# Neos-codes/microbeast

Measured on AMD Instinct MI355X. Metric: env frames/sec (whole node) on 16x16 microRTS, higher is better.
Workload: dtype bf16

## Files before the change

### microbeast_amd/_native.py

```python
from __future__ import annotations

import ctypes
import importlib.util
import os
import sys
import threading
from pathlib import Path

import torch

_LIB = Path(__file__).resolve().parent / "_lib"
_lock = threading.Lock()
_kern = None
_rt = None

c_void_p, c_int, c_int64, c_float = ctypes.c_void_p, ctypes.c_int, ctypes.c_int64, ctypes.c_float

_SIGS = {
    "mbk_multi_copy": [c_void_p, c_int, c_void_p],
    "mbk_comm_standin": [c_void_p, c_void_p, c_int64, c_int, c_int, c_void_p],
    "mbk_row_gather": [c_void_p, c_void_p, c_void_p, c_int, c_int64, c_void_p],
    "mbk_memset": [c_void_p, c_int, c_int64, c_void_p],
    "mbk_masked_cell_fwd": [c_void_p, c_int, c_void_p, c_void_p, c_void_p, c_int, c_int64,
                            c_void_p, c_void_p, c_void_p],
# ... 53 lines not shown
    "mbk_set_learner_occupancy": [c_int, c_int],
    "mbk_set_work_queues": [c_int],
    "mbk_set_work_queue_site": [c_int, c_int],
    "mbk_conv0_row_set": [c_int],
    "mbk_fc_wgrad_parts": [c_int, c_int, c_int],
    "mbk_fc_wgrad": [c_void_p, c_void_p, c_int, c_int, c_int, c_void_p, c_int, c_void_p, c_int,
                     c_void_p],
    "mbk_fc_fwd": [c_void_p, c_int, c_void_p, c_void_p, c_void_p, c_void_p, c_int, c_int, c_int,
                   c_void_p, c_void_p, c_void_p],
    "mbk_gemm_nt": [c_void_p, c_void_p, c_void_p, c_void_p, c_int, c_int, c_int, c_int, c_int,
                    c_int, c_int, c_int, c_int, c_void_p],
    "mbk_wgrad_reduce": [c_void_p, c_int, c_int, c_int, c_int, c_void_p, c_void_p, c_int,
                         c_void_p],
    "mbk_wgrad_reduce_batch": [c_void_p, c_int, c_void_p],
    "mbk_pool_bwd": [c_void_p, c_void_p, c_int, c_int, c_int, c_int, c_void_p, c_void_p],
    "mbk_conv_pack": [c_void_p, c_int, c_void_p],
    "mbk_head_compact": [c_void_p, c_int, c_int, c_void_p, c_void_p, c_void_p, c_void_p,
                         c_void_p, c_void_p, c_void_p, c_void_p, c_void_p, c_void_p, c_void_p,
                         c_void_p, c_void_p, c_int, c_void_p, c_void_p, c_void_p, c_void_p],
    "mbk_head_fwd": [c_void_p, c_void_p, c_void_p, c_void_p, c_void_p, c_void_p, c_int,
                     c_void_p, c_void_p, c_void_p, c_void_p, c_void_p, c_void_p, c_int, c_int,
                     c_void_p, c_void_p, c_int, c_void_p],
    "mbk_fc_wgrad_wide_parts": [c_int, c_int, c_int],
    "mbk_fc_wgrad_wide": [c_void_p, c_void_p, c_int, c_int, c_int, c_int, c_void_p, c_int,
                          c_void_p, c_void_p, c_void_p],
    "mbk_head_score": [c_void_p, c_void_p, c_void_p, c_void_p, c_void_p, c_void_p, c_void_p,
                       c_void_p, c_void_p, c_void_p, c_void_p, c_int, c_void_p, c_void_p,
                       c_void_p, c_void_p],
    "mbk_head_pair_rowsum": [c_void_p, c_void_p, c_int, c_int, c_void_p, c_void_p, c_void_p,
                             c_void_p, c_void_p],
    "mbk_head_bwd": [c_void_p, c_void_p, c_void_p, c_void_p, c_void_p, c_void_p, c_void_p,
                     c_void_p, c_void_p, c_void_p, c_void_p, c_void_p, c_void_p, c_void_p,
                     c_void_p, c_int, c_int, c_void_p, c_void_p, c_void_p, c_void_p,
                     c_void_p, c_void_p, c_void_p],
    "mbk_head_dx_gather": [c_void_p, c_void_p, c_void_p, c_int, c_int, c_void_p, c_void_p],
    "mbk_head_dx_value_parts": [c_int],
    "mbk_head_dx_value": [c_void_p, c_void_p, c_void_p, c_int, c_int, c_void_p, c_void_p,
                          c_void_p, c_int, c_void_p, c_void_p, c_int, c_void_p],
    "mbk_head_pack": [c_void_p, c_void_p, c_int, c_void_p, c_void_p, c_void_p, c_void_p],
    "mbk_decode_obs_mask": [c_void_p, c_void_p, c_int, c_int, c_int, c_void_p, c_void_p, c_void_p],
    "mbk_decode_obs_mask_bucket": [c_void_p, c_void_p, c_int, c_int, c_int, c_void_p, c_void_p,
                                   c_void_p, c_void_p, c_void_p, c_void_p, c_void_p],
    "mbk_head_units": [c_void_p, c_int, c_int, c_void_p, c_void_p, c_void_p, c_void_p, c_void_p,
                       c_void_p],
    "mbk_row_sum_rng": [c_void_p, c_int64, c_int, c_void_p, c_void_p, c_void_p],
    "mbk_row_sum_pack": [c_void_p, c_int64, c_int, c_void_p, c_void_p, c_void_p, c_void_p,
                         c_void_p, c_int, c_void_p],
    "mbk_head_fwd_counts": [c_void_p, c_void_p, c_void_p, c_void_p, c_void_p, c_void_p,
                            c_void_p, c_void_p, c_int, c_int, c_int, c_void_p, c_void_p],
    "mbk_trunk_tail": [c_void_p, c_void_p, c_void_p, c_int, c_int, c_int, c_void_p, c_void_p],
    "mbk_trunk_tail_fp8": [c_void_p, c_void_p, c_void_p, c_void_p, c_int, c_int, c_int, c_void_p,
                           c_void_p],
    "mbk_trunk_tail_fc": [c_void_p, c_void_p, c_void_p, c_int, c_int, c_int, c_void_p, c_void_p,
                          c_void_p, c_void_p, c_void_p, c_int, c_void_p, c_void_p, c_void_p],
    "mbk_pack_env_actions": [c_void_p, c_int64, c_void_p, c_void_p],
    "mbk_res_bwd16_parts": [c_int, c_int, c_int, c_int],
    "mbk_res_bwd32_parts": [c_int, c_int, c_int, c_int],
    "mbk_res_bwd32_partial_floats": [c_int],
    "mbk_res_bwd32": [c_void_p, c_void_p, c_void_p, c_void_p, c_void_p, c_void_p, c_void_p, c_int,
                      c_void_p, c_void_p, c_void_p, c_void_p, c_int, c_int, c_int, c_int,
                      c_int, c_void_p],
    "mbk_res_fwd16": [c_void_p, c_void_p, c_void_p, c_void_p, c_void_p, c_void_p, c_void_p, c_int,
                      c_int, c_int, c_int, c_void_p],
    "mbk_res_fwd16_stage": [c_void_p, c_void_p, c_void_p, c_void_p, c_void_p, c_void_p, c_void_p,
                            c_void_p, c_void_p, c_void_p, c_void_p, c_int, c_int, c_int, c_int,
                            c_void_p],
    "mbk_res_blk32_fwd": [c_void_p, c_void_p, c_void_p, c_void_p, c_void_p, c_int, c_int, c_int, c_int,
# ... 118 lines not shown
```

### microbeast_amd/csrc/kernels/head.hip

```cpp
#include <cstdio>
#include <vector>

#include "../include/mbk_api.h"
#include "../include/microrts_rules.h"
#include "common.h"

#ifndef MBK_HA_MB
#define MBK_HA_MB 4
#endif

using namespace mbk;

typedef __bf16 bf16x8 __attribute__((ext_vector_type(8)));
typedef short s16x4 __attribute__((ext_vector_type(4)));
typedef float f32x4 __attribute__((ext_vector_type(4)));
typedef __hip_bfloat16 bf16;

namespace {

constexpr int KD = 256;
constexpr int NP = 80;
constexpr int NPT = 96;

union Frag8 {
// ... 510 lines not shown
  }
}
__global__ __launch_bounds__(64 * HA_NW, 2) void head_act_kernel(HeadActArgs a) {
  head_act_kernel_body(a);
}

__global__ __launch_bounds__(256) void head_pair_rowsum_kernel(const int* __restrict__ pidx,
                                                               const uint32_t* __restrict__ abits,
                                                               int F,
                                                               int S, const float* __restrict__ plp,
                                                               const float* __restrict__ pent,
                                                               float* __restrict__ logp,
                                                               float* __restrict__ ent) {
  const int f = blockIdx.x * 256 + threadIdx.x;
  if (f >= F) return;
  const int SW = abits_words(S);
  const uint32_t* ab = abits + (size_t)f * SW;
  const int* pr = pidx + (size_t)f * S;
  float a = 0.f, b = 0.f;
  for (int w = 0; w < SW; ++w) {
    uint32_t bits = ab[w];
    if (32 * w + 32 > S) bits &= (1u << (S - 32 * w)) - 1u;
    while (bits) {
      const int p = pr[32 * w + __builtin_ctz(bits)];
      bits &= bits - 1u;
      a += plp[p];
      if (pent) b += pent[p];
    }
  }
  logp[f] = a;
  if (ent) ent[f] = b;
}

constexpr int HB_NW = 8;
constexpr int HB_TM = 16 * HB_NW;
constexpr int HB_RX = 544, HB_RW = 544, HB_RZ = 288;
constexpr int HB_LW = 0, HB_LX = 96 * HB_RW, HB_LZ = HB_LX + HB_TM * HB_RX;
constexpr int HB_LB = HB_LZ + HB_TM * HB_RZ;
constexpr int HB_LDS = HB_LB + HB_NW * NP * 4;

__device__ __forceinline__ int hb_phi(int r) {
  const int b = (r >> 2) & 3;
  return (b == 1 || b == 2) ? r ^ 12 : r;
}
template <int CTRL>
__device__ __forceinline__ float hb_dpp(float v) {
  return __int_as_float(__builtin_amdgcn_mov_dpp(__float_as_int(v), CTRL, 0xF, 0xF, true));
}
constexpr int kHbDpp[4] = {0xB1, 0x4E, 0x141, 0x140};
template <int N>
__device__ __forceinline__ void hb_max16(float (&v)[N]) {
#pragma unroll
  for (int st = 0; st < 4; ++st)
#pragma unroll
    for (int j = 0; j < N; ++j) {
      const float o = st == 0 ? hb_dpp<0xB1>(v[j]) : st == 1 ? hb_dpp<0x4E>(v[j])
                    : st == 2 ? hb_dpp<0x141>(v[j]) : hb_dpp<0x140>(v[j]);
      v[j] = fmaxf(v[j], o);
    }
}
template <int N>
__device__ __forceinline__ void hb_sum16(float (&v)[N]) {
#pragma unroll
  for (int st = 0; st < 4; ++st)
#pragma unroll
    for (int j = 0; j < N; ++j) {
      const float o = st == 0 ? hb_dpp<0xB1>(v[j]) : st == 1 ? hb_dpp<0x4E>(v[j])
                    : st == 2 ? hb_dpp<0x141>(v[j]) : hb_dpp<0x140>(v[j]);
      v[j] += o;
    }
}

template <bool ST>
__global__ __launch_bounds__(64 * HB_NW, 1) void head_bwd2_kernel(
    const bf16* __restrict__ X, const bf16* __restrict__ Wp, const float* __restrict__ bp,
    const uint32_t* __restrict__ mask, const uint8_t* __restrict__ action,
    const int* __restrict__ pairs, const int* __restrict__ grp_start,
    const int* __restrict__ grp_count, const int* __restrict__ chunk_cell,
    const int* __restrict__ chunk_row, const int* __restrict__ totals,
    const float* __restrict__ g_logp, const float* __restrict__ g_ent, int S,
    bf16* __restrict__ dXp, float* __restrict__ dWp, float* __restrict__ dbp,
    uint64_t* __restrict__ stamps, const float* __restrict__ stats) {
  extern __shared__ __attribute__((aligned(16))) char smem[];
  char* wl = smem + HB_LW;
  int nst = 0;
#define HB_STAMP(k)                                                                        \
  do {                                                                                     \
    if (stamps && threadIdx.x == 0 && nst < 8)                                             \
      stamps[((size_t)blockIdx.x * 8 + nst) * 8 + (k)] = __builtin_amdgcn_s_memrealtime(); \
  } while (0)
  char* xl = smem + HB_LX;
  char* zl = smem + HB_LZ;
  float* bl = (float*)(smem + HB_LB);
  const int tid = threadIdx.x, lane = tid & 63, wave = tid >> 6;
  const int G = lane >> 4, li = lane & 15;
  const int nchunks = totals[2];
  const int qn = (nchunks + (int)gridDim.x - 1) / (int)gridDim.x;
  const int ch_begin = (int)blockIdx.x * qn, ch_end = min(nchunks, ch_begin + qn);
  if (ch_begin >= nchunks) return;
  for (int e = tid; e < 16 * HB_RW / 16; e += 64 * HB_NW)
    ((uint4*)(wl + 80 * HB_RW))[e] = make_uint4(0, 0, 0, 0);

  int sk[5], so[5];
#pragma unroll
  for (int nb = 0; nb < 5; ++nb) {
    const int col = nb * 16 + li;
    int k = 0;
#pragma unroll
    for (int q = 1; q < kComps; ++q) k += col >= seg_off(q) ? 1 : 0;
    sk[nb] = col < kCell ? k : kComps;
    so[nb] = col - seg_off(k);
  }

  const int sq = tid & 31, sr0 = tid >> 5;
  uint4 xr[8];
  struct Cur {
    int ch, t0, c, g0, n;
  };
  auto chunk_cur = [&](int ch) {
    if (ch >= ch_end) ch = nchunks;
    Cur u{ch, 0, 0, 0, 0};
    if (ch < nchunks) {
      u.c = chunk_cell[ch];
      u.g0 = chunk_row[ch];
      u.n = min(CHUNK, grp_start[u.c] + grp_count[u.c] - u.g0);
    }
    return u;
  };
  auto advance = [&](const Cur& u) {
    if (u.ch >= nchunks) return u;
    if (u.t0 + HB_TM < u.n) return Cur{u.ch, u.t0 + HB_TM, u.c, u.g0, u.n};
    return chunk_cur(u.ch + 1);
  };
  const int mrow = tid / 3, mpart = tid - 3 * (tid / 3);
  int fx[8], fr = -1;
  uint32_t mt[3] = {0u, 0u, 0u};
  auto load_fx = [&](const Cur& u) {
    const int nr = u.ch < nchunks ? min(HB_TM, u.n - u.t0) : 0;
#pragma unroll
    for (int k = 0; k < 8; ++k) fx[k] = sr0 + 16 * k < nr ? pairs[u.g0 + u.t0 + sr0 + 16 * k] : -1;
    fr = tid < 3 * HB_TM && mrow < nr ? pairs[u.g0 + u.t0 + mrow] : -1;
  };
  auto load_meta = [&](int c) {
    mt[0] = mt[1] = mt[2] = 0u;
    if (fr < 0) {
      if (mpart == 2) mt[2] = 0xFFFFFFFFu;
      return;
    }
    const size_t fc = (size_t)fr * S + c;
    if (mpart == 0) {
      mt[0] = mask[fc * 3]; mt[1] = mask[fc * 3 + 1]; mt[2] = mask[fc * 3 + 2];
    } else if (mpart == 1) {
      const size_t ab0 = fc * kComps;
      const uint32_t* aw4 = (const uint32_t*)(action + (ab0 & ~(size_t)3));
      mt[0] = aw4[0]; mt[1] = aw4[1]; mt[2] = (ab0 & 3) >= 2 ? aw4[2] : 0u;
    } else {
      mt[0] = __float_as_uint(g_logp[fr]);
      mt[1] = g_ent ? __float_as_uint(g_ent[fr]) : 0u;
      mt[2] = (uint32_t)fr;
    }
  };
  auto store_meta = [&]() {
    if (tid < 3 * HB_TM) {
      uint32_t* d = (uint32_t*)(zl + hb_phi(mrow) * HB_RZ + 192 + mpart * 12);
      d[0] = mt[0]; d[1] = mt[1]; d[2] = mt[2];
    }
  };
  const int srow = tid >> 2, squ = tid & 3;
  uint4 st4 = make_uint4(0u, 0u, 0u, 0u);
  auto load_stats = [&](const Cur& u) {
    if constexpr (ST) {
      const int nr = u.ch < nchunks ? min(HB_TM, u.n - u.t0) : 0;
      st4 = srow < nr ? ((const uint4*)(stats + (size_t)(u.g0 + u.t0 + srow) * 16))[squ]
                      : make_uint4(0u, 0u, 0u, 0u);
    }
  };
  auto store_stats = [&]() {
    if constexpr (ST) {
      uint32_t* d = (uint32_t*)(zl + hb_phi(srow) * HB_RZ + 228 + squ * 16);
      d[0] = st4.x; d[1] = st4.y;
      if (squ < 3) {
        d[2] = st4.z; d[3] = st4.w;
      }
    }
  };
  auto load_x = [&]() {
#pragma unroll
    for (int k = 0; k < 8; ++k)
      xr[k] = fx[k] >= 0 ? ((const uint4*)(X + (size_t)fx[k] * KD))[sq] : make_uint4(0, 0, 0, 0);
  };
  auto store_x = [&]() {
#pragma unroll
    for (int k = 0; k < 8; ++k) *(uint4*)(xl + hb_phi(sr0 + 16 * k) * HB_RX + sq * 16) = xr[k];
  };
  auto stage_w = [&](int c) {
    const uint4* src = (const uint4*)(Wp + (size_t)c * NP * KD);
    uint4 v[5];
#pragma unroll
    for (int k = 0; k < 5; ++k) v[k] = src[(sr0 + 16 * k) * (KD / 8) + sq];
#pragma unroll
    for (int k = 0; k < 5; ++k) *(uint4*)(wl + hb_phi(sr0 + 16 * k) * HB_RW + sq * 16) = v[k];
  };

  Cur cur = chunk_cur(ch_begin);
  Cur nx1 = advance(cur);
  load_fx(cur);
  load_x();
  load_meta(cur.c);
  load_stats(cur);
  load_fx(nx1);
  f32x4 accw[5][2];
  float dbs[5], bcol[5];
  bool new_chunk = true;
  for (;;) {
    const int ch = cur.ch, c = cur.c, g = cur.g0 + cur.t0, nr = min(HB_TM, cur.n - cur.t0);
    HB_STAMP(0);
    lds_barrier();
    store_x();
    store_meta();
    store_stats();
    if (new_chunk) {
      stage_w(c);
#pragma unroll
      for (int mb = 0; mb < 5; ++mb)
#pragma unroll
        for (int nb = 0; nb < 2; ++nb) accw[mb][nb] = f32x4{0.f, 0.f, 0.f, 0.f};
#pragma unroll
      for (int nb = 0; nb < 5; ++nb) {
        dbs[nb] = 0.f;
        bcol[nb] = bp[(size_t)c * NP + nb * 16 + li];
      }
      new_chunk = false;
    }
    lds_barrier();
    HB_STAMP(1);
    const bool last = nx1.ch != ch, has_next = nx1.ch < nchunks;
    const bool run_end = last && !(has_next && nx1.c == c);
    f32x4 z[5];
#pragma unroll
    for (int nb = 0; nb < 5; ++nb) z[nb] = f32x4{0.f, 0.f, 0.f, 0.f};
    const char* xa = xl + hb_phi(16 * wave + li) * HB_RX + 16 * G;
#pragma unroll 2
    for (int ks = 0; ks < KD / 32; ++ks) {
      Frag8 a;
      a.u = *(const uint4*)(xa + ks * 64);
#pragma unroll
      for (int nb = 0; nb < 5; ++nb) {
        Frag8 b;
        b.u = *(const uint4*)(wl + hb_phi(nb * 16 + li) * HB_RW + ks * 64 + 16 * G);
        z[nb] = __builtin_amdgcn_mfma_f32_16x16x32_bf16(a.v, b.v, z[nb], 0, 0, 0);
      }
    }

    HB_STAMP(2);
    uint32_t mw[4][3], aw[4][3];
    int ab[4];
    float gl[4], ge[4];
#pragma unroll
    for (int i = 0; i < 4; ++i) {
      const uint32_t* m = (const uint32_t*)(zl + hb_phi(16 * wave + 4 * G + i) * HB_RZ + 192);
      const uint4 q0 = *(const uint4*)m, q1 = *(const uint4*)(m + 4);
      const uint32_t fw = m[8];
      mw[i][0] = q0.x; mw[i][1] = q0.y; mw[i][2] = q0.z;
      aw[i][0] = q0.w; aw[i][1] = q1.x; aw[i][2] = q1.y;
      gl[i] = __uint_as_float(q1.z);
      ge[i] = __uint_as_float(q1.w);
      ab[i] = (int)((((size_t)(int)fw * S + c) * kComps) & 3);
    }
    uint32_t okm = 0u;
    float zz[5][4];
#pragma unroll
    for (int nb = 0; nb < 5; ++nb) {
      const float b = bcol[nb];
#pragma unroll
      for (int i = 0; i < 4; ++i) {
        zz[nb][i] = z[nb][i] + b;
        const int bit = (nb & 1) * 16 + li;
        okm |= (sk[nb] < kComps && ((mw[i][nb >> 1] >> bit) & 1u)) ? 1u << (nb * 4 + i) : 0u;
      }
    }
    if constexpr (ST) {
#pragma unroll
      for (int i = 0; i < 4; ++i) {
        const char* rowp = zl + hb_phi(16 * wave + 4 * G + i) * HB_RZ;
#pragma unroll
        for (int nb = 0; nb < 5; ++nb) {
          const int k = min(sk[nb], kComps - 1);
          const float lse = *(const float*)(rowp + 228 + 4 * k);
          const float H = *(const float*)(rowp + 256 + 4 * k);
          const int bi = ab[i] + k;
          const uint32_t wsel = bi < 4 ? aw[i][0] : bi < 8 ? aw[i][1] : aw[i][2];
          const int a = (int)((wsel >> (8 * (bi & 3))) & 0xFFu);
          const float lp = zz[nb][i] - lse;
          const float p = __expf(lp);
          zz[nb][i] = gl[i] * ((so[nb] == a ? 1.f : 0.f) - p) - ge[i] * p * (lp + H);
        }
      }
    }
#pragma unroll
    for (int k = 0; k < (ST ? 0 : kComps); ++k) {
      const int c0 = seg_off(k), c1 = seg_off(k + 1);
      const int nb0 = c0 / 16, nb1 = (c1 - 1) / 16;
      bool any = false;
#pragma unroll
      for (int nb = nb0; nb <= nb1; ++nb)
#pragma unroll
        for (int i = 0; i < 4; ++i) any |= ((okm >> (nb * 4 + i)) & 1u) && sk[nb] == k;
      if (__ballot(any) == 0ull) continue;
      float mx[4], sm[8];
#pragma unroll
      for (int i = 0; i < 4; ++i) {
        mx[i] = -INFINITY;
#pragma unroll
        for (int nb = nb0; nb <= nb1; ++nb)
          if (((okm >> (nb * 4 + i)) & 1u) && sk[nb] == k) mx[i] = fmaxf(mx[i], zz[nb][i]);
      }
      hb_max16(mx);
#pragma unroll
      for (int i = 0; i < 4; ++i) {
        float e_s = 0.f, e_sz = 0.f;
#pragma unroll
        for (int nb = nb0; nb <= nb1; ++nb) {
          const bool in = ((okm >> (nb * 4 + i)) & 1u) && sk[nb] == k;
          const float e = in ? __expf(zz[nb][i] - mx[i]) : 0.f;
          e_s += e;
          e_sz += e * zz[nb][i];
        }
        sm[2 * i] = e_s;
        sm[2 * i + 1] = e_sz;
// ... 9 lines not shown
#pragma unroll
        for (int nb = nb0; nb <= nb1; ++nb) {
          const bool in = ((okm >> (nb * 4 + i)) & 1u) && sk[nb] == k;
          const float lp = zz[nb][i] - lse;
          const float p = __expf(lp);
          const float v = gl[i] * ((so[nb] == a ? 1.f : 0.f) - p) - ge[i] * p * (lp + H);
          zz[nb][i] = in ? v : zz[nb][i];
        }
      }
    }
    float d[5][4];
#pragma unroll
    for (int nb = 0; nb < 5; ++nb)
#pragma unroll
      for (int i = 0; i < 4; ++i) d[nb][i] = ((okm >> (nb * 4 + i)) & 1u) ? zz[nb][i] : 0.f;
#pragma unroll
    for (int nb = 0; nb < 5; ++nb) {
      float cs = 0.f;
#pragma unroll
      for (int i = 0; i < 4; ++i) {
        const int r = 16 * wave + 4 * G + i;
        *(bf16*)(zl + hb_phi(r) * HB_RZ + (nb * 16 + li) * 2) = f2bf(d[nb][i]);
        cs += d[nb][i];
      }
      dbs[nb] += cs;
    }
    if (li < 8) {
#pragma unroll
      for (int i = 0; i < 4; ++i) {
        const int r = 16 * wave + 4 * G + i;
        *(uint32_t*)(zl + hb_phi(r) * HB_RZ + 160 + li * 4) = 0u;
      }
    }
    if (has_next) {
      load_x();
      load_meta(nx1.c);
      load_stats(nx1);
    }
    const Cur nx2 = advance(nx1);
    if (nx2.ch < nchunks) load_fx(nx2);
    HB_STAMP(3);
    lds_barrier();
    HB_STAMP(4);

#pragma unroll 1
    for (int ks = 0; ks < HB_TM / 32; ++ks) {
      Frag8 a[5];
#pragma unroll
      for (int mb = 0; mb < 5; ++mb)
#pragma unroll
        for (int h = 0; h < 2; ++h) {
          const int pr = hb_phi(ks * 32 + 8 * G + 4 * h + (li >> 2));
          a[mb].h[h] = tr_read(zl + pr * HB_RZ + (mb * 16 + 4 * (li & 3)) * 2);
        }
#pragma unroll
      for (int nb = 0; nb < 2; ++nb) {
        Frag8 b;
#pragma unroll
        for (int h = 0; h < 2; ++h) {
          const int pr = hb_phi(ks * 32 + 8 * G + 4 * h + (li >> 2));
          b.h[h] = tr_read(xl + pr * HB_RX + (32 * wave + nb * 16 + 4 * (li & 3)) * 2);
        }
#pragma unroll
        for (int mb = 0; mb < 5; ++mb)
          accw[mb][nb] = __builtin_amdgcn_mfma_f32_16x16x32_bf16(a[mb].v, b.v, accw[mb][nb], 0, 0, 0);
      }
    }
    lds_barrier();
    HB_STAMP(5);
    const char* za = zl + hb_phi(16 * wave + li) * HB_RZ + 16 * G;
    char* stg = xl + wave * 16 * 528;
#pragma unroll 1
    for (int hc = 0; hc < 2; ++hc) {
      f32x4 acc[8];
#pragma unroll
      for (int nb = 0; nb < 8; ++nb) acc[nb] = f32x4{0.f, 0.f, 0.f, 0.f};
#pragma unroll 1
      for (int ks = 0; ks < NPT / 32; ++ks) {
        Frag8 a;
        a.u = *(const uint4*)(za + ks * 64);
#pragma unroll
        for (int nb = 0; nb < 8; ++nb) {
          Frag8 b;
#pragma unroll
          for (int h = 0; h < 2; ++h) {
            const int kr = ks * 32 + 8 * G + 4 * h + (li >> 2);
            b.h[h] = tr_read(wl + hb_phi(kr) * HB_RW + ((hc * 8 + nb) * 16 + 4 * (li & 3)) * 2);
          }
          acc[nb] = __builtin_amdgcn_mfma_f32_16x16x32_bf16(a.v, b.v, acc[nb], 0, 0, 0);
        }
      }
#pragma unroll
      for (int i = 0; i < 4; ++i)
#pragma unroll
        for (int nb = 0; nb < 8; ++nb)
          *(bf16*)(stg + (4 * G + i) * 528 + ((hc * 8 + nb) * 16 + li) * 2) = f2bf(acc[nb][i]);
    }
    asm volatile("s_waitcnt vmcnt(0)" ::: "memory");
#pragma unroll
    for (int q = 0; q < 8; ++q) {
      const int rr = 2 * q + (lane >> 5), r = 16 * wave + rr;
      const uint4 v = *(const uint4*)(stg + rr * 528 + (lane & 31) * 16);
      if (r < nr) *(uint4*)(dXp + (size_t)(g + r) * KD + (lane & 31) * 8) = v;
    }
    HB_STAMP(6);
    if (run_end) {
      float* dwb = dWp + ((size_t)ch * kCell + 4 * G) * KD + 32 * wave + li;
#pragma unroll
      for (int mb = 0; mb < 5; ++mb)
#pragma unroll
        for (int i = 0; i < 4; ++i) {
          if (mb == 4 && 4 * G + i >= kCell - 64) continue;
#pragma unroll
          for (int nb = 0; nb < 2; ++nb) dwb[(mb * 16 + i) * KD + nb * 16] = accw[mb][nb][i];
        }
#pragma unroll
      for (int nb = 0; nb < 5; ++nb) {
        float v = dbs[nb];
        v += __shfl_xor(v, 16, 64);
        v += __shfl_xor(v, 32, 64);
        if (G == 0) bl[wave * NP + nb * 16 + li] = v;
      }
      lds_barrier();
      if (tid < kCell) {
        float v = 0.f;
        for (int w = 0; w < HB_NW; ++w) v += bl[w * NP + tid];
        dbp[(size_t)ch * kCell + tid] = v;
      }
      if (!has_next) break;
      new_chunk = true;
    }
    HB_STAMP(7);
    ++nst;
    cur = nx1;
    nx1 = nx2;
  }
}

constexpr int HS_NW = 4, HS_TM = 64 * HS_NW, HS_IPC = CHUNK / HS_TM;
constexpr int HS_ZS = NP + 1;
constexpr int HS_LZ = 80 * HB_RW;
constexpr int HS_LDS = HS_LZ + HS_NW * 64 * HS_ZS * 4;

__global__ __launch_bounds__(64 * HS_NW, 1) void head_score_kernel(
    const bf16* __restrict__ X, const bf16* __restrict__ Wp, const float* __restrict__ bp,
    const uint32_t* __restrict__ mask, const uint8_t* __restrict__ action,
    const int* __restrict__ pairs, const int* __restrict__ grp_start,
// ... 380 lines not shown
                     (const bf16*)Wp, bp, mask, action, rng, sample, pairs, unit_cell, unit_row,
                     grp_start, grp_count, totals, S, cell_lp, cell_ent, pair_out,
                     (const int*)nullptr, 0);
  return (int)hipGetLastError();
}

extern "C" int mbk_head_fwd_counts(const void* X, const void* Wp, const float* bp,
                                   const uint32_t* mask, uint8_t* action, const uint64_t* rng,
                                   const int* bucket, const int* cnt, int E, int S, int grid,
                                   float* cell_lp, hipStream_t stream) {
  if (S < 1 || S > kMaxUnitCells - 1 || !cnt) return (int)hipErrorInvalidValue;
  hipLaunchKernelGGL(head_fwd_kernel, dim3(grid), dim3(256), 0, stream, (const bf16*)X,
                     (const bf16*)Wp, bp, mask, action, rng, 1, bucket, (const int*)nullptr,
                     (const int*)nullptr, (const int*)nullptr, (const int*)nullptr,
                     (const int*)nullptr, S, cell_lp, (float*)nullptr, 0, cnt, E);
  return (int)hipGetLastError();
}

extern "C" int mbk_head_pair_rowsum(const int* pidx, const uint32_t* abits, int F, int S,
                                    const float* plp, const float* pent, float* logp, float* ent,
                                    hipStream_t stream) {
  if (F <= 0) return 0;
  hipLaunchKernelGGL(head_pair_rowsum_kernel, dim3((F + 255) / 256), dim3(256), 0, stream, pidx,
                     abits, F, S, plp, pent, logp, ent);
  return (int)hipGetLastError();
}

extern "C" int mbk_head_bwd(const void* X, const void* Wp, const void* WpT, const float* bp,
                            const uint32_t* mask, const uint8_t* action, const int* pairs,
                            const int* grp_start, const int* grp_count, const int* chunk_cell,
                            const int* chunk_row, const int* chunk_start, const int* totals,
                            const float* g_logp, const float* g_ent, int S, int grid, void* dXp,
                            float* dWp, float* dbp, float* dW, float* db, const float* stats,
                            hipStream_t stream) {
  int bwd_grid = 1;
  {
    static int cus = 0;
    static uint64_t* hb_stamps = nullptr;
    if (!cus) {
      int dev = 0;
      hipGetDevice(&dev);
      hipDeviceGetAttribute(&cus, hipDeviceAttributeMultiprocessorCount, dev);
      if (cus <= 0) cus = 256;
      hipFuncSetAttribute((const void*)head_bwd2_kernel<false>,
                          hipFuncAttributeMaxDynamicSharedMemorySize, HB_LDS);
      hipFuncSetAttribute((const void*)head_bwd2_kernel<true>,
                          hipFuncAttributeMaxDynamicSharedMemorySize, HB_LDS);
      if (getenv("MBK_HB_STAMPS")) {
        hipMalloc(&hb_stamps, (size_t)cus * 64 * 8);
        hipMemset(hb_stamps, 0, (size_t)cus * 64 * 8);
      }
    }
    const int g2 = std::max(1, std::min(grid, cus));
    bwd_grid = g2;
    hipLaunchKernelGGL(stats ? head_bwd2_kernel<true> : head_bwd2_kernel<false>, dim3(g2),
                       dim3(64 * HB_NW), HB_LDS, stream, (const bf16*)X, (const bf16*)Wp, bp,
                       mask, action, pairs, grp_start, grp_count, chunk_cell, chunk_row, totals,
                       g_logp, g_ent, S, (bf16*)dXp, dWp, dbp, hb_stamps, stats);
    if (hb_stamps) {
      std::vector<uint64_t> h((size_t)g2 * 64);
      hipMemcpyAsync(h.data(), hb_stamps, h.size() * 8, hipMemcpyDeviceToHost, stream);
      hipStreamSynchronize(stream);
      double acc[8] = {0};
      int n = 0;
      for (int b = 0; b < g2; ++b)
        for (int t = 1; t < 8; ++t) {
          const uint64_t* r = &h[((size_t)b * 8 + t) * 8];
          if (!r[0] || !r[7]) continue;
          for (int k = 0; k < 7; ++k) acc[k] += (double)(r[k + 1] - r[k]) * 0.01;
          ++n;
        }
      fprintf(stderr, "head_bwd2 phases (us, %d tiles): store+W %.2f | loads+Z %.2f | dZ %.2f | "
              "B2 %.2f | dX %.2f | dW %.2f | end %.2f\n", n, acc[0] / n, acc[1] / n, acc[2] / n,
              acc[3] / n, acc[4] / n, acc[5] / n, acc[6] / n);
      hipMemsetAsync(hb_stamps, 0, h.size() * 8, stream);
    }
  }
  dim3 g2((kCell * KD + kCell + 255) / 256, S);
  hipLaunchKernelGGL(head_dw_reduce_kernel, g2, dim3(256), 0, stream, dWp, dbp, chunk_start,
                     grp_count, totals, bwd_grid, S, dW, db);
  return (int)hipGetLastError();
}

extern "C" int mbk_head_score(const void* X, const void* Wp, const float* bp,
                              const uint32_t* mask, const uint8_t* action, const int* pairs,
                              const int* grp_start, const int* grp_count, const int* chunk_cell,
                              const int* chunk_row, const int* totals, int S, float* plp,
                              float* pent, float* stats, hipStream_t stream) {
  static int cus = 0;
  if (!cus) {
    int dev = 0;
// ... 98 lines not shown
```

### microbeast_amd/ops/head.py

```python
from __future__ import annotations


import torch

from .. import _native as N

KD, NP, NPT = 256, 80, 96


class SparseHead:
    def __init__(self, S: int, device: torch.device):
        self.S = S
        self.device = device
        self.Wp = torch.zeros(S, NP, KD, dtype=torch.bfloat16, device=device)
        self.WpT = torch.zeros(S, KD, NPT, dtype=torch.bfloat16, device=device)
        self.bp = torch.zeros(S, NP, dtype=torch.float32, device=device)
        self.totals = torch.zeros(3, dtype=torch.int32, device=device)
        self.chunk_start = torch.zeros(S, dtype=torch.int32, device=device)
        self.grp_start = torch.zeros(S, dtype=torch.int32, device=device)
        self.grp_count = torch.zeros(S, dtype=torch.int32, device=device)
        self._F = -1
        n_cu = torch.cuda.get_device_properties(device).multi_processor_count if device.type == "cuda" else 1
        self.fwd_grid = 2 * n_cu
        self.count_units = True
        self.score_tiles = True
        self.score_stats = True
        self.stats = None
        self._fwd_totals = None
        self._prep = None

    def _ensure(self, F: int):
        if F <= self._F:
            return
        S, dev = self.S, self.device
        fb = min(256, max(8, F // 64))
        nfb = (F + fb - 1) // fb
        self.cnt = torch.zeros(S * nfb, dtype=torch.int32, device=dev)
        self.off = torch.zeros(S * nfb, dtype=torch.int32, device=dev)
        self.unit_cell = torch.zeros(F * S // 16 + S + 1, dtype=torch.int32, device=dev)
        self.unit_row = torch.zeros_like(self.unit_cell)
        self.chunk_cell = torch.zeros(F * S // 512 + S + 1, dtype=torch.int32, device=dev)
        self.chunk_row = torch.zeros_like(self.chunk_cell)
        self.pairs = torch.zeros(F * S, dtype=torch.int32, device=dev)
        self.pidx = torch.zeros(F * S, dtype=torch.int32, device=dev)
        self.abits = torch.zeros(F * ((S + 31) // 32), dtype=torch.int32, device=dev)
        self.cell_lp = torch.zeros(F * S, dtype=torch.float32, device=dev)
        self.cell_ent = torch.zeros(F * S, dtype=torch.float32, device=dev)
        self._F = F

    def ensure_buckets(self, E: int):
        self._ensure(E)
        if getattr(self, "_bucket_E", -1) != E:
            self.bucket_cnt = torch.zeros(self.S, dtype=torch.int32, device=self.device)
            self.bucket = torch.zeros(self.S * E, dtype=torch.int32, device=self.device)
            self._bucket_E = E

    def sample_bucketed(self, X: torch.Tensor, mask_bits: torch.Tensor, action: torch.Tensor,
                        rng: torch.Tensor, logp_out: torch.Tensor,
                        act16_out: torch.Tensor | None = None) -> torch.Tensor:
# ... 112 lines not shown
                                   self.fwd_grid, self.cell_lp.data_ptr(),
                                   self.cell_ent.data_ptr() if want_ent else None,
                                   int(pair_out), st), "head_fwd")
        logp = logp_out if logp_out is not None else torch.empty(F, dtype=torch.float32, device=X.device)
        ent = None
        if want_ent:
            ent = ent_out if ent_out is not None else torch.empty(F, dtype=torch.float32, device=X.device)
        if pair_out:
            N.check(k.mbk_head_pair_rowsum(self.pidx.data_ptr(), self._abits.data_ptr(), F,
                                           self.S,
                                           self.cell_lp.data_ptr(),
                                           self.cell_ent.data_ptr() if want_ent else None,
                                           logp.data_ptr(), N.ptr(ent), st), "head_pair_rowsum")
        else:
            N.check(k.mbk_row_sum(self.cell_lp.data_ptr(), F, self.S, logp.data_ptr(), st),
                    "row_sum")
            if want_ent:
                N.check(k.mbk_row_sum(self.cell_ent.data_ptr(), F, self.S, ent.data_ptr(), st),
                        "row_sum")
        if sample:
            N.check(k.mbk_rng_advance(rng.data_ptr(), st), "rng_advance")
        return logp, ent

    def backward(self, X, mask_bits, action, g_logp, g_ent, dW=None, db=None, value=None):
        F = X.shape[0]
        k = N.kernels()
        st = N.stream_ptr()
        fwd = self._fwd_totals
        if fwd is not None:
            P, nch = fwd
        else:
            P, _, nch = (int(v) for v in self.totals.tolist())
        dXp = torch.empty(max(P, 1), KD, dtype=torch.bfloat16, device=X.device)
        dWp = torch.empty(max(nch, 1), 78, KD, dtype=torch.float32, device=X.device)
        dbp = torch.empty(max(nch, 1), 78, dtype=torch.float32, device=X.device)
        if dW is None:
            dW = torch.empty(self.S * 78, KD, dtype=torch.float32, device=X.device)
        if db is None:
            db = torch.empty(self.S * 78, dtype=torch.float32, device=X.device)
        assert dW.is_contiguous() and db.is_contiguous() and dW.numel() == self.S * 78 * KD
        grid = max(1, min(nch, self.fwd_grid))
        N.check(k.mbk_head_bwd(X.data_ptr(), self.Wp.data_ptr(), self.WpT.data_ptr(),
                               self.bp.data_ptr(), mask_bits.data_ptr(), action.data_ptr(),
                               self.pairs.data_ptr(), self.grp_start.data_ptr(),
                               self.grp_count.data_ptr(), self.chunk_cell.data_ptr(),
                               self.chunk_row.data_ptr(), self.chunk_start.data_ptr(),
                               self.totals.data_ptr(), g_logp.data_ptr(), N.ptr(g_ent), self.S,
                               grid, dXp.data_ptr(), dWp.data_ptr(), dbp.data_ptr(),
                               dW.data_ptr(), db.data_ptr(),
                               self.stats.data_ptr() if fwd is not None else None, st),
                "head_bwd")
        if value is not None:
            dv, h, wc, partial = value
            R = h.shape[0]
            assert h.is_contiguous() and h.shape[1] == KD and dv.dtype == torch.float32
            dh = torch.empty(R, KD, dtype=torch.bfloat16, device=X.device)
            N.check(k.mbk_head_dx_value(dXp.data_ptr(), self.pidx.data_ptr(),
                                        self._abits.data_ptr(), F, self.S,
                                        dv.data_ptr(), h.data_ptr(), wc.data_ptr(), R,
                                        dh.data_ptr(), partial.data_ptr(), partial.shape[0], st),
                    "head_dx_value")
            return dh, dW, db
        dX = torch.empty(F, KD, dtype=torch.float32, device=X.device)
        N.check(k.mbk_head_dx_gather(dXp.data_ptr(), self.pidx.data_ptr(), self._abits.data_ptr(),
                                     F, self.S, dX.data_ptr(), st), "head_dx_gather")
        return dX, dW, db


class _SparseHeadScore(torch.autograd.Function):
    @staticmethod
    def forward(ctx, X, W, b, mask_bits, action, head: SparseHead):
        Xc = X.contiguous()
        head.pack(W.detach(), b.detach(), with_t=True)
        logp, ent = head.forward(Xc, mask_bits, action, sample=False, rng=None)
        ctx.head = head
        ctx.save_for_backward(Xc, mask_bits, action)
        ctx.x_dtype = X.dtype
        return logp, ent

    @staticmethod
    def backward(ctx, g_logp, g_ent):
        Xc, mask_bits, action = ctx.saved_tensors
        F = Xc.shape[0]
# ... 29 lines not shown
```

Before: 20.35 million.

## Add 64-pair 4-wave head backward tile with half-width weight staging

```diff
diff --git a/microbeast_amd/_native.py b/microbeast_amd/_native.py
--- a/microbeast_amd/_native.py
+++ b/microbeast_amd/_native.py
@@ -109,7 +109,7 @@
     "mbk_head_bwd": [c_void_p, c_void_p, c_void_p, c_void_p, c_void_p, c_void_p, c_void_p,
                      c_void_p, c_void_p, c_void_p, c_void_p, c_void_p, c_void_p, c_void_p,
                      c_void_p, c_int, c_int, c_void_p, c_void_p, c_void_p, c_void_p,
-                     c_void_p, c_void_p, c_void_p],
+                     c_void_p, c_void_p, c_int, c_void_p],
     "mbk_head_dx_gather": [c_void_p, c_void_p, c_void_p, c_int, c_int, c_void_p, c_void_p],
     "mbk_head_dx_value_parts": [c_int],
     "mbk_head_dx_value": [c_void_p, c_void_p, c_void_p, c_int, c_int, c_void_p, c_void_p,
diff --git a/microbeast_amd/csrc/kernels/head.hip b/microbeast_amd/csrc/kernels/head.hip
--- a/microbeast_amd/csrc/kernels/head.hip
+++ b/microbeast_amd/csrc/kernels/head.hip
@@ -566,12 +566,22 @@
   if (ent) ent[f] = b;
 }
 
-constexpr int HB_NW = 8;
-constexpr int HB_TM = 16 * HB_NW;
 constexpr int HB_RX = 544, HB_RW = 544, HB_RZ = 288;
-constexpr int HB_LW = 0, HB_LX = 96 * HB_RW, HB_LZ = HB_LX + HB_TM * HB_RX;
-constexpr int HB_LB = HB_LZ + HB_TM * HB_RZ;
-constexpr int HB_LDS = HB_LB + HB_NW * NP * 4;
+template <int NW>
+struct HbCfg {
+  static_assert(NW == 8 || NW == 4, "head_bwd2: 128-pair (8 waves) or 64-pair (4 waves) tiles");
+  static constexpr bool WH = NW == 4;
+  static constexpr int TM = 16 * NW;
+  static constexpr int RW = WH ? 288 : HB_RW;
+  static constexpr int RS = 2 * NW;
+  static constexpr int NBW = 16 / NW;
+  static constexpr int LW = 0, LX = (WH ? 80 : 96) * RW, LZ = LX + TM * HB_RX;
+  static constexpr int LB = LZ + TM * HB_RZ;
+  static constexpr int LDS = LB + NW * NP * 4;
+  static constexpr int WGS = WH ? 2 : 1;
+};
+static_assert(HbCfg<4>::LDS <= 78 * 1024, "64-pair form: beside launch A's 80 KB in a CU");
+constexpr int HB_LDS = HbCfg<8>::LDS;
 
 __device__ __forceinline__ int hb_phi(int r) {
   const int b = (r >> 2) & 3;
@@ -605,8 +615,8 @@
     }
 }
 
-template <bool ST>
-__global__ __launch_bounds__(64 * HB_NW, 1) void head_bwd2_kernel(
+template <bool ST, int NW>
+__global__ __launch_bounds__(64 * NW, HbCfg<NW>::WGS) void head_bwd2_kernel(
     const bf16* __restrict__ X, const bf16* __restrict__ Wp, const float* __restrict__ bp,
     const uint32_t* __restrict__ mask, const uint8_t* __restrict__ action,
     const int* __restrict__ pairs, const int* __restrict__ grp_start,
@@ -615,6 +625,10 @@
     const float* __restrict__ g_logp, const float* __restrict__ g_ent, int S,
     bf16* __restrict__ dXp, float* __restrict__ dWp, float* __restrict__ dbp,
     uint64_t* __restrict__ stamps, const float* __restrict__ stats) {
+  using Cfg = HbCfg<NW>;
+  constexpr bool WH = Cfg::WH;
+  constexpr int HB_NW = NW, HB_TM = Cfg::TM, HB_RW = Cfg::RW, HB_RS = Cfg::RS, HB_NBW = Cfg::NBW;
+  constexpr int HB_LW = Cfg::LW, HB_LX = Cfg::LX, HB_LZ = Cfg::LZ, HB_LB = Cfg::LB;
   extern __shared__ __attribute__((aligned(16))) char smem[];
   char* wl = smem + HB_LW;
   int nst = 0;
@@ -626,27 +640,31 @@
   char* xl = smem + HB_LX;
   char* zl = smem + HB_LZ;
   float* bl = (float*)(smem + HB_LB);
-  const int tid = threadIdx.x, lane = tid & 63, wave = tid >> 6;
-  const int G = lane >> 4, li = lane & 15;
+  int tid = threadIdx.x, lane = tid & 63, wave = tid >> 6;
+  int G = lane >> 4, li = lane & 15;
   const int nchunks = totals[2];
   const int qn = (nchunks + (int)gridDim.x - 1) / (int)gridDim.x;
   const int ch_begin = (int)blockIdx.x * qn, ch_end = min(nchunks, ch_begin + qn);
   if (ch_begin >= nchunks) return;
-  for (int e = tid; e < 16 * HB_RW / 16; e += 64 * HB_NW)
-    ((uint4*)(wl + 80 * HB_RW))[e] = make_uint4(0, 0, 0, 0);
+  if constexpr (!WH)
+    for (int e = tid; e < 16 * HB_RW / 16; e += 64 * HB_NW)
+      ((uint4*)(wl + 80 * HB_RW))[e] = make_uint4(0, 0, 0, 0);
 
   int sk[5], so[5];
-#pragma unroll
-  for (int nb = 0; nb < 5; ++nb) {
-    const int col = nb * 16 + li;
-    int k = 0;
-#pragma unroll
-    for (int q = 1; q < kComps; ++q) k += col >= seg_off(q) ? 1 : 0;
-    sk[nb] = col < kCell ? k : kComps;
-    so[nb] = col - seg_off(k);
-  }
-
-  const int sq = tid & 31, sr0 = tid >> 5;
+  auto seg_cols = [&]() {
+#pragma unroll
+    for (int nb = 0; nb < 5; ++nb) {
+      const int col = nb * 16 + li;
+      int k = 0;
+#pragma unroll
+      for (int q = 1; q < kComps; ++q) k += col >= seg_off(q) ? 1 : 0;
+      sk[nb] = col < kCell ? k : kComps;
+      so[nb] = col - seg_off(k);
+    }
+  };
+  seg_cols();
+
+  int sq = tid & 31, sr0 = tid >> 5;
   uint4 xr[8];
   struct Cur {
     int ch, t0, c, g0, n;
@@ -666,13 +684,14 @@
     if (u.t0 + HB_TM < u.n) return Cur{u.ch, u.t0 + HB_TM, u.c, u.g0, u.n};
     return chunk_cur(u.ch + 1);
   };
-  const int mrow = tid / 3, mpart = tid - 3 * (tid / 3);
+  int mrow = tid / 3, mpart = tid - 3 * (tid / 3);
   int fx[8], fr = -1;
   uint32_t mt[3] = {0u, 0u, 0u};
   auto load_fx = [&](const Cur& u) {
     const int nr = u.ch < nchunks ? min(HB_TM, u.n - u.t0) : 0;
 #pragma unroll
-    for (int k = 0; k < 8; ++k) fx[k] = sr0 + 16 * k < nr ? pairs[u.g0 + u.t0 + sr0 + 16 * k] : -1;
+    for (int k = 0; k < 8; ++k)
+      fx[k] = sr0 + HB_RS * k < nr ? pairs[u.g0 + u.t0 + sr0 + HB_RS * k] : -1;
     fr = tid < 3 * HB_TM && mrow < nr ? pairs[u.g0 + u.t0 + mrow] : -1;
   };
   auto load_meta = [&](int c) {
@@ -700,7 +719,7 @@
       d[0] = mt[0]; d[1] = mt[1]; d[2] = mt[2];
     }
   };
-  const int srow = tid >> 2, squ = tid & 3;
+  int srow = tid >> 2, squ = tid & 3;
   uint4 st4 = make_uint4(0u, 0u, 0u, 0u);
   auto load_stats = [&](const Cur& u) {
     if constexpr (ST) {
@@ -725,7 +744,7 @@
   };
   auto store_x = [&]() {
 #pragma unroll
-    for (int k = 0; k < 8; ++k) *(uint4*)(xl + hb_phi(sr0 + 16 * k) * HB_RX + sq * 16) = xr[k];
+    for (int k = 0; k < 8; ++k) *(uint4*)(xl + hb_phi(sr0 + HB_RS * k) * HB_RX + sq * 16) = xr[k];
   };
   auto stage_w = [&](int c) {
     const uint4* src = (const uint4*)(Wp + (size_t)c * NP * KD);
@@ -735,7 +754,38 @@
 #pragma unroll
     for (int k = 0; k < 5; ++k) *(uint4*)(wl + hb_phi(sr0 + 16 * k) * HB_RW + sq * 16) = v[k];
   };
-
+  int hq = tid & 15, hr0 = tid >> 4;
+  uint4 wv0, wv1, wv2, wv3, wv4;
+  wv0 = wv1 = wv2 = wv3 = wv4 = make_uint4(0u, 0u, 0u, 0u);
+  auto load_wh = [&](int c, int hf) {
+    const uint4* src = (const uint4*)(Wp + (size_t)c * NP * KD) + hr0 * (KD / 8) + hf * 16 + hq;
+    wv0 = src[0 * 16 * (KD / 8)];
+    wv1 = src[1 * 16 * (KD / 8)];
+    wv2 = src[2 * 16 * (KD / 8)];
+    wv3 = src[3 * 16 * (KD / 8)];
+    wv4 = src[4 * 16 * (KD / 8)];
+  };
+  auto store_wh = [&]() {
+    char* d = wl + hb_phi(hr0) * HB_RW + hq * 16;
+    *(uint4*)(d + 0 * 16 * HB_RW) = wv0;
+    *(uint4*)(d + 1 * 16 * HB_RW) = wv1;
+    *(uint4*)(d + 2 * 16 * HB_RW) = wv2;
+    *(uint4*)(d + 3 * 16 * HB_RW) = wv3;
+    *(uint4*)(d + 4 * 16 * HB_RW) = wv4;
+  };
+
+  auto reindex = [&]() {
+    if constexpr (WH) {
+      int t = threadIdx.x;
+      asm volatile("" : "+v"(t));
+      tid = t; lane = t & 63; wave = t >> 6;
+      G = lane >> 4; li = lane & 15;
+      sq = t & 31; sr0 = t >> 5;
+      mrow = t / 3; mpart = t - 3 * (t / 3);
+      srow = t >> 2; squ = t & 3;
+      hq = t & 15; hr0 = t >> 4;
+    }
+  };
   Cur cur = chunk_cur(ch_begin);
   Cur nx1 = advance(cur);
   load_fx(cur);
@@ -743,22 +793,28 @@
   load_meta(cur.c);
   load_stats(cur);
   load_fx(nx1);
-  f32x4 accw[5][2];
+  f32x4 accw[5][HB_NBW];
   float dbs[5], bcol[5];
   bool new_chunk = true;
   for (;;) {
     const int ch = cur.ch, c = cur.c, g = cur.g0 + cur.t0, nr = min(HB_TM, cur.n - cur.t0);
     HB_STAMP(0);
     lds_barrier();
+    reindex();
     store_x();
     store_meta();
     store_stats();
     if (new_chunk) {
-      stage_w(c);
+      if constexpr (WH) {
+        load_wh(c, 0);
+        store_wh();
+      } else {
+        stage_w(c);
+      }
 #pragma unroll
       for (int mb = 0; mb < 5; ++mb)
 #pragma unroll
-        for (int nb = 0; nb < 2; ++nb) accw[mb][nb] = f32x4{0.f, 0.f, 0.f, 0.f};
+        for (int nb = 0; nb < HB_NBW; ++nb) accw[mb][nb] = f32x4{0.f, 0.f, 0.f, 0.f};
 #pragma unroll
       for (int nb = 0; nb < 5; ++nb) {
         dbs[nb] = 0.f;
@@ -766,6 +822,7 @@
       }
       new_chunk = false;
     }
+    if constexpr (WH) load_wh(c, 1);
     lds_barrier();
     HB_STAMP(1);
     const bool last = nx1.ch != ch, has_next = nx1.ch < nchunks;
@@ -773,20 +830,45 @@
     f32x4 z[5];
 #pragma unroll
     for (int nb = 0; nb < 5; ++nb) z[nb] = f32x4{0.f, 0.f, 0.f, 0.f};
+    reindex();
     const char* xa = xl + hb_phi(16 * wave + li) * HB_RX + 16 * G;
+    if constexpr (!WH) {
 #pragma unroll 2
-    for (int ks = 0; ks < KD / 32; ++ks) {
-      Frag8 a;
-      a.u = *(const uint4*)(xa + ks * 64);
-#pragma unroll
-      for (int nb = 0; nb < 5; ++nb) {
-        Frag8 b;
-        b.u = *(const uint4*)(wl + hb_phi(nb * 16 + li) * HB_RW + ks * 64 + 16 * G);
-        z[nb] = __builtin_amdgcn_mfma_f32_16x16x32_bf16(a.v, b.v, z[nb], 0, 0, 0);
+      for (int ks = 0; ks < KD / 32; ++ks) {
+        Frag8 a;
+        a.u = *(const uint4*)(xa + ks * 64);
+#pragma unroll
+        for (int nb = 0; nb < 5; ++nb) {
+          Frag8 b;
+          b.u = *(const uint4*)(wl + hb_phi(nb * 16 + li) * HB_RW + ks * 64 + 16 * G);
+          z[nb] = __builtin_amdgcn_mfma_f32_16x16x32_bf16(a.v, b.v, z[nb], 0, 0, 0);
+        }
+      }
+    } else {
+#pragma unroll 1
+      for (int hf = 0; hf < 2; ++hf) {
+        if (hf) {
+          lds_barrier();
+          store_wh();
+          lds_barrier();
+        }
+#pragma unroll 2
+        for (int ks = 0; ks < KD / 64; ++ks) {
+          Frag8 a;
+          a.u = *(const uint4*)(xa + hf * (KD / 64) * 64 + ks * 64);
+#pragma unroll
+          for (int nb = 0; nb < 5; ++nb) {
+            Frag8 b;
+            b.u = *(const uint4*)(wl + hb_phi(nb * 16 + li) * HB_RW + ks * 64 + 16 * G);
+            z[nb] = __builtin_amdgcn_mfma_f32_16x16x32_bf16(a.v, b.v, z[nb], 0, 0, 0);
+          }
+        }
       }
     }
 
     HB_STAMP(2);
+    reindex();
+    if constexpr (WH) seg_cols();
     uint32_t mw[4][3], aw[4][3];
     int ab[4];
     float gl[4], ge[4];
@@ -829,6 +911,7 @@
           const float p = __expf(lp);
           zz[nb][i] = gl[i] * ((so[nb] == a ? 1.f : 0.f) - p) - ge[i] * p * (lp + H);
         }
+        __builtin_amdgcn_sched_barrier(0);
       }
     }
 #pragma unroll
@@ -904,16 +987,19 @@
         *(uint32_t*)(zl + hb_phi(r) * HB_RZ + 160 + li * 4) = 0u;
       }
     }
+    reindex();
     if (has_next) {
       load_x();
       load_meta(nx1.c);
       load_stats(nx1);
     }
+    if constexpr (WH) load_wh(c, 0);
     const Cur nx2 = advance(nx1);
     if (nx2.ch < nchunks) load_fx(nx2);
     HB_STAMP(3);
     lds_barrier();
     HB_STAMP(4);
+    reindex();
 
 #pragma unroll 1
     for (int ks = 0; ks < HB_TM / 32; ++ks) {
@@ -926,12 +1012,12 @@
           a[mb].h[h] = tr_read(zl + pr * HB_RZ + (mb * 16 + 4 * (li & 3)) * 2);
         }
 #pragma unroll
-      for (int nb = 0; nb < 2; ++nb) {
+      for (int nb = 0; nb < HB_NBW; ++nb) {
         Frag8 b;
 #pragma unroll
         for (int h = 0; h < 2; ++h) {
           const int pr = hb_phi(ks * 32 + 8 * G + 4 * h + (li >> 2));
-          b.h[h] = tr_read(xl + pr * HB_RX + (32 * wave + nb * 16 + 4 * (li & 3)) * 2);
+          b.h[h] = tr_read(xl + pr * HB_RX + (16 * HB_NBW * wave + nb * 16 + 4 * (li & 3)) * 2);
         }
 #pragma unroll
         for (int mb = 0; mb < 5; ++mb)
@@ -940,10 +1026,17 @@
     }
     lds_barrier();
     HB_STAMP(5);
+    reindex();
     const char* za = zl + hb_phi(16 * wave + li) * HB_RZ + 16 * G;
     char* stg = xl + wave * 16 * 528;
 #pragma unroll 1
-    for (int hc = 0; hc < 2; ++hc) {
+    for (int hi = 0; hi < 2; ++hi) {
+      const int hc = WH ? 1 - hi : hi;
+      if (WH && hi) {
+        lds_barrier();
+        store_wh();
+        lds_barrier();
+      }
       f32x4 acc[8];
 #pragma unroll
       for (int nb = 0; nb < 8; ++nb) acc[nb] = f32x4{0.f, 0.f, 0.f, 0.f};
@@ -956,8 +1049,10 @@
           Frag8 b;
 #pragma unroll
           for (int h = 0; h < 2; ++h) {
-            const int kr = ks * 32 + 8 * G + 4 * h + (li >> 2);
-            b.h[h] = tr_read(wl + hb_phi(kr) * HB_RW + ((hc * 8 + nb) * 16 + 4 * (li & 3)) * 2);
+            int kr = ks * 32 + 8 * G + 4 * h + (li >> 2);
+            if (WH && kr >= 80) kr -= 16;
+            b.h[h] = tr_read(wl + hb_phi(kr) * HB_RW +
+                             (((WH ? 0 : hc * 8) + nb) * 16 + 4 * (li & 3)) * 2);
           }
           acc[nb] = __builtin_amdgcn_mfma_f32_16x16x32_bf16(a.v, b.v, acc[nb], 0, 0, 0);
         }
@@ -977,14 +1072,15 @@
     }
     HB_STAMP(6);
     if (run_end) {
-      float* dwb = dWp + ((size_t)ch * kCell + 4 * G) * KD + 32 * wave + li;
+      reindex();
+      float* dwb = dWp + ((size_t)ch * kCell + 4 * G) * KD + 16 * HB_NBW * wave + li;
 #pragma unroll
       for (int mb = 0; mb < 5; ++mb)
 #pragma unroll
         for (int i = 0; i < 4; ++i) {
           if (mb == 4 && 4 * G + i >= kCell - 64) continue;
 #pragma unroll
-          for (int nb = 0; nb < 2; ++nb) dwb[(mb * 16 + i) * KD + nb * 16] = accw[mb][nb][i];
+          for (int nb = 0; nb < HB_NBW; ++nb) dwb[(mb * 16 + i) * KD + nb * 16] = accw[mb][nb][i];
         }
 #pragma unroll
       for (int nb = 0; nb < 5; ++nb) {
@@ -1431,31 +1527,53 @@
                             const int* chunk_row, const int* chunk_start, const int* totals,
                             const float* g_logp, const float* g_ent, int S, int grid, void* dXp,
                             float* dWp, float* dbp, float* dW, float* db, const float* stats,
-                            hipStream_t stream) {
+                            int tile, hipStream_t stream) {
+  if (tile != 64 && tile != 128) return (int)hipErrorInvalidValue;
   int bwd_grid = 1;
   {
-    static int cus = 0;
+    static int cus = 0, wgs64 = 0;
     static uint64_t* hb_stamps = nullptr;
     if (!cus) {
       int dev = 0;
       hipGetDevice(&dev);
       hipDeviceGetAttribute(&cus, hipDeviceAttributeMultiprocessorCount, dev);
       if (cus <= 0) cus = 256;
-      hipFuncSetAttribute((const void*)head_bwd2_kernel<false>,
-                          hipFuncAttributeMaxDynamicSharedMemorySize, HB_LDS);
-      hipFuncSetAttribute((const void*)head_bwd2_kernel<true>,
-                          hipFuncAttributeMaxDynamicSharedMemorySize, HB_LDS);
+      hipFuncSetAttribute((const void*)head_bwd2_kernel<false, 8>,
+                          hipFuncAttributeMaxDynamicSharedMemorySize, HbCfg<8>::LDS);
+      hipFuncSetAttribute((const void*)head_bwd2_kernel<true, 8>,
+                          hipFuncAttributeMaxDynamicSharedMemorySize, HbCfg<8>::LDS);
+      hipFuncSetAttribute((const void*)head_bwd2_kernel<false, 4>,
+                          hipFuncAttributeMaxDynamicSharedMemorySize, HbCfg<4>::LDS);
+      hipFuncSetAttribute((const void*)head_bwd2_kernel<true, 4>,
+                          hipFuncAttributeMaxDynamicSharedMemorySize, HbCfg<4>::LDS);
+      int occ = 0, occ0 = 0;
+      if (hipOccupancyMaxActiveBlocksPerMultiprocessor(&occ, (const void*)head_bwd2_kernel<true, 4>,
+                                                       64 * 4, HbCfg<4>::LDS) != hipSuccess ||
+          hipOccupancyMaxActiveBlocksPerMultiprocessor(&occ0,
+                                                       (const void*)head_bwd2_kernel<false, 4>,
+                                                       64 * 4, HbCfg<4>::LDS) != hipSuccess)
+        occ = occ0 = 0;
+      wgs64 = std::max(1, std::min(std::min(occ, occ0), HbCfg<4>::WGS));
       if (getenv("MBK_HB_STAMPS")) {
-        hipMalloc(&hb_stamps, (size_t)cus * 64 * 8);
-        hipMemset(hb_stamps, 0, (size_t)cus * 64 * 8);
-      }
-    }
-    const int g2 = std::max(1, std::min(grid, cus));
+        hipMalloc(&hb_stamps, (size_t)cus * HbCfg<4>::WGS * 64 * 8);
+        hipMemset(hb_stamps, 0, (size_t)cus * HbCfg<4>::WGS * 64 * 8);
+      }
+    }
+    const int g2 = std::max(1, std::min(grid, tile == 64 ? cus * mbk_occ_b(wgs64) : cus));
     bwd_grid = g2;
-    hipLaunchKernelGGL(stats ? head_bwd2_kernel<true> : head_bwd2_kernel<false>, dim3(g2),
-                       dim3(64 * HB_NW), HB_LDS, stream, (const bf16*)X, (const bf16*)Wp, bp,
-                       mask, action, pairs, grp_start, grp_count, chunk_cell, chunk_row, totals,
-                       g_logp, g_ent, S, (bf16*)dXp, dWp, dbp, hb_stamps, stats);
+    auto launch = [&](auto kern, int nw, int lds) {
+      hipLaunchKernelGGL(kern, dim3(g2), dim3(64 * nw), lds, stream, (const bf16*)X,
+                         (const bf16*)Wp, bp, mask, action, pairs, grp_start, grp_count,
+                         chunk_cell, chunk_row, totals, g_logp, g_ent, S, (bf16*)dXp, dWp, dbp,
+                         hb_stamps, stats);
+    };
+    if (tile == 64) {
+      if (stats) launch(head_bwd2_kernel<true, 4>, 4, HbCfg<4>::LDS);
+      else launch(head_bwd2_kernel<false, 4>, 4, HbCfg<4>::LDS);
+    } else {
+      if (stats) launch(head_bwd2_kernel<true, 8>, 8, HbCfg<8>::LDS);
+      else launch(head_bwd2_kernel<false, 8>, 8, HbCfg<8>::LDS);
+    }
     if (hb_stamps) {
       std::vector<uint64_t> h((size_t)g2 * 64);
       hipMemcpyAsync(h.data(), hb_stamps, h.size() * 8, hipMemcpyDeviceToHost, stream);
diff --git a/microbeast_amd/ops/head.py b/microbeast_amd/ops/head.py
--- a/microbeast_amd/ops/head.py
+++ b/microbeast_amd/ops/head.py
@@ -25,6 +25,8 @@
         self.count_units = True
         self.score_tiles = True
         self.score_stats = True
+        self.bwd_tile = 64
+        self.keep_pair_rows = False
         self.stats = None
         self._fwd_totals = None
         self._prep = None
@@ -203,6 +205,8 @@
         else:
             P, _, nch = (int(v) for v in self.totals.tolist())
         dXp = torch.empty(max(P, 1), KD, dtype=torch.bfloat16, device=X.device)
+        if self.keep_pair_rows:
+            self.dXp = dXp
         dWp = torch.empty(max(nch, 1), 78, KD, dtype=torch.float32, device=X.device)
         dbp = torch.empty(max(nch, 1), 78, dtype=torch.float32, device=X.device)
         if dW is None:
@@ -219,7 +223,8 @@
                                self.totals.data_ptr(), g_logp.data_ptr(), N.ptr(g_ent), self.S,
                                grid, dXp.data_ptr(), dWp.data_ptr(), dbp.data_ptr(),
                                dW.data_ptr(), db.data_ptr(),
-                               self.stats.data_ptr() if fwd is not None else None, st),
+                               self.stats.data_ptr() if fwd is not None else None,
+                               self.bwd_tile, st),
                 "head_bwd")
         if value is not None:
             dv, h, wc, partial = value
```

New measurement: 19.58 million. 0.962x the previous value.
